# rostin79s/TFHE-AES

Hardware: AMD Instinct MI355X
Metric: AES-128 CTR blocks/sec (FHE) (higher is better)
Workload: dtype u64+f64; 1 GPU; configs[2]: 128 CTR blocks per GPU, Server::aes_encrypt 10 rounds (1280 bit-CBS/block), counters pre-incremented client-side; params=PARAM_OPT, blocks_per_gpu=128, total_blocks=128

## Files before the change

include/fheaes.h:

```cpp
#ifndef FHEAES_H
#define FHEAES_H

#include <stddef.h>
#include <stdint.h>

#ifdef __cplusplus
extern "C" {
#endif

#define FHEAES_OK 0
#define FHEAES_ERR_INVALID -1
#define FHEAES_ERR_NOKEYS -2
#define FHEAES_ERR_DEVICE -3
#define FHEAES_ERR_NOMEM -4

#define FHEAES_HOST 0
#define FHEAES_DEVICE 1

typedef struct fheaes_params {
    uint32_t lwe_dimension;
    uint32_t glwe_dimension;
    uint32_t polynomial_size;
    uint32_t pbs_base_log;
    uint32_t pbs_level;
// ... 224 lines not shown
int fheaes_get_twiddles(double *psi_out);
int fheaes_read_bsk_fourier(fheaes_ctx *ctx, uint32_t i, double *out);
int fheaes_k2_launch_plan(uint64_t m, uint32_t cu_count, uint32_t k, int *form, uint64_t *units_main, uint32_t *r_main,
                          uint64_t *units_tail, uint32_t *r_tail);
int fheaes_k2_launch_plan_forms(uint64_t m, uint32_t cu_count, uint32_t k, int allow_pair, int *form, uint64_t *units_main, uint32_t *r_main,
                                uint64_t *units_tail, uint32_t *r_tail);
int fheaes_k2_context_plan(fheaes_ctx *ctx, uint64_t m, int *form, uint64_t *units_main, uint32_t *r_main, uint64_t *units_tail,
                           uint32_t *r_tail, char *kernel, size_t kernel_cap);
int fheaes_k2_set_parking(fheaes_ctx *ctx, int claimed);
int fheaes_k2_set_forms(fheaes_ctx *ctx, int allow_pair, int allow_home);
int fheaes_aes_window_plan(uint64_t n_blocks, uint32_t steps, uint32_t cu_count, uint32_t k, uint64_t *window_blocks, uint64_t *launches,
                           uint64_t *generations, uint64_t *generations_by_round);
int fheaes_aes_context_window(fheaes_ctx *ctx, uint64_t n_blocks, uint32_t steps, uint64_t *window_blocks);
#define FHEAES_AES_WINDOW_OFF 0xFFFFFFFFu
int fheaes_aes_set_window(fheaes_ctx *ctx, uint32_t window_blocks);
#define FHEAES_K2_PARK_SLOTS 1024
int fheaes_k2_park_debug(fheaes_ctx *ctx, const uint32_t *initial_owner, int record);
int fheaes_k2_park_read(fheaes_ctx *ctx, uint64_t *fallbacks, uint64_t *violations, uint32_t *owner_out, uint32_t *record_out,
                        uint64_t record_cap, uint64_t *record_n);
#define FHEAES_WS_BUFFERS 17
#define FHEAES_WS_F64 0
#define FHEAES_WS_WORDS 1
#define FHEAES_WS_TABLES 2
#define FHEAES_WS_PATTERN_F64_HALF 0x7FF87FF8u
#define FHEAES_WS_PATTERN_WORDS 0xA5
#define FHEAES_WS_PATTERN_TABLES 1u
#define FHEAES_WS_POISON_FILL 0
#define FHEAES_WS_POISON_RELEASE 1
int fheaes_workspace_info(fheaes_ctx *ctx, uint32_t index, char *name_out, size_t name_cap, uint64_t *bytes_out, int *class_out,
                          uint64_t *first_word_out, uint64_t *last_word_out);
// ... 9 lines not shown
```

tfhe_aes_amd/_native.py:

```python
from __future__ import annotations

import ctypes
import os
import re
from pathlib import Path

import numpy as np

from . import _build
from .params import CParams, WopbsParameters

HOST, DEVICE = 0, 1
MAC_NONE = 0xFFFFFFFF
KW_MIN_SEMIBLOCKS, KW_MAX_SEMIBLOCKS, KW_MAX_KEYS = 2, 8, 4096
AES_WINDOW_OFF = 0xFFFFFFFF
GATE_LWE, GATE_GLWE = 0, 1
K2_PARK_SLOTS = 1024
AUDIT_MAX_ROWS, AUDIT_RECORDS = 256, 16
WS_BUFFERS = 17
WS_CLASSES = ("f64", "words", "tables")
WS_POISON_FILL, WS_POISON_RELEASE = 0, 1
STAGES = ("keyswitch", "blind_rotate", "pfpks", "ggsw_fft", "vertical_packing", "linear")
AUDIT_STAGES = ("keyswitch", "blind_rotate", "pfpks")

_u64p = ctypes.POINTER(ctypes.c_uint64)
_dp = ctypes.POINTER(ctypes.c_double)
_u32p = ctypes.POINTER(ctypes.c_uint32)
_u8p = ctypes.POINTER(ctypes.c_uint8)
_ctx = ctypes.c_void_p
_c = ctypes
# ... 108 lines not shown
    "fheaes_profile_reset": (_c.c_int, [_ctx]),
    "fheaes_profile_read": (_c.c_int, [_ctx, _c.c_int, _dp, _u64p, _u64p]),
    "fheaes_get_twiddles": (_c.c_int, [_dp]),
    "fheaes_read_bsk_fourier": (_c.c_int, [_ctx, _c.c_uint32, _dp]),
    "fheaes_k2_launch_plan": (_c.c_int, [_c.c_uint64, _c.c_uint32, _c.c_uint32, _c.POINTER(_c.c_int), _c.POINTER(_c.c_uint64), _c.POINTER(_c.c_uint32),
                                       _c.POINTER(_c.c_uint64), _c.POINTER(_c.c_uint32)]),
    "fheaes_k2_launch_plan_forms": (_c.c_int, [_c.c_uint64, _c.c_uint32, _c.c_uint32, _c.c_int, _c.POINTER(_c.c_int), _c.POINTER(_c.c_uint64),
                                             _c.POINTER(_c.c_uint32), _c.POINTER(_c.c_uint64), _c.POINTER(_c.c_uint32)]),
    "fheaes_k2_context_plan": (_c.c_int, [_ctx, _c.c_uint64, _c.POINTER(_c.c_int), _c.POINTER(_c.c_uint64), _c.POINTER(_c.c_uint32),
                                        _c.POINTER(_c.c_uint64), _c.POINTER(_c.c_uint32), _c.c_char_p, _c.c_size_t]),
    "fheaes_k2_set_parking": (_c.c_int, [_ctx, _c.c_int]),
    "fheaes_k2_set_forms": (_c.c_int, [_ctx, _c.c_int, _c.c_int]),
    "fheaes_aes_window_plan": (_c.c_int, [_c.c_uint64, _c.c_uint32, _c.c_uint32, _c.c_uint32, _u64p, _u64p, _u64p, _u64p]),
    "fheaes_aes_context_window": (_c.c_int, [_ctx, _c.c_uint64, _c.c_uint32, _u64p]),
    "fheaes_aes_set_window": (_c.c_int, [_ctx, _c.c_uint32]),
    "fheaes_k2_park_debug": (_c.c_int, [_ctx, _c.POINTER(_c.c_uint32), _c.c_int]),
    "fheaes_k2_park_read": (_c.c_int, [_ctx, _u64p, _u64p, _c.POINTER(_c.c_uint32), _c.POINTER(_c.c_uint32), _c.c_uint64, _u64p]),
    "fheaes_audit_set": (_c.c_int, [_ctx, _c.c_uint32, _c.c_uint64, _c.c_uint64]),
    "fheaes_audit_rows": (_c.c_int, [_c.c_uint64, _c.c_uint64, _c.c_uint64, _c.c_uint32, _u64p]),
    "fheaes_audit_read": (_c.c_int, [_ctx, _u64p, _u64p, _u64p, _u64p, _c.c_uint64, _u64p]),
    "fheaes_audit_debug": (_c.c_int, [_ctx, _c.c_uint64, _c.c_uint32, _c.c_uint64]),
    "fheaes_audit_stage_set": (_c.c_int, [_ctx, _c.c_int, _c.c_uint32, _c.c_uint64, _c.c_uint64]),
    "fheaes_audit_stage_read": (_c.c_int, [_ctx, _c.c_int, _u64p, _u64p, _u64p, _u64p, _c.c_uint64, _u64p]),
    "fheaes_audit_stage_debug": (_c.c_int, [_ctx, _c.c_int, _c.c_uint64, _c.c_uint32, _c.c_uint64]),
    "fheaes_audit_plain_batch": (_c.c_int, [_ctx, _c.c_int, _c.c_void_p, _c.c_uint64, _c.c_int, _c.c_void_p]),
    "fheaes_workspace_info": (_c.c_int, [_ctx, _c.c_uint32, _c.c_char_p, _c.c_size_t, _u64p, _c.POINTER(_c.c_int), _u64p, _u64p]),
    "fheaes_workspace_poison": (_c.c_int, [_ctx, _c.c_int, _u64p]),
    "fheaes_alloc_debug": (_c.c_int, [_ctx, _c.c_uint64, _u64p]),
    "fheaes_version": (_c.c_char_p, []),
}
# ... 443 lines not shown

    def k2_set_parking(self, claimed: bool):
        self._check(self._lib.fheaes_k2_set_parking(self._h, 1 if claimed else 0))

    def k2_set_forms(self, allow_pair: bool = True, allow_home: bool = True):
        self._check(self._lib.fheaes_k2_set_forms(self._h, 1 if allow_pair else 0, 1 if allow_home else 0))

    def aes_window(self, n_blocks: int, steps: int) -> int:
        w = _c.c_uint64()
        self._check(self._lib.fheaes_aes_context_window(self._h, n_blocks, steps, _c.byref(w)))
        return w.value

    def aes_set_window(self, window_blocks: int = 0):
        self._check(self._lib.fheaes_aes_set_window(self._h, int(window_blocks)))

    def k2_park_debug(self, initial=None, record: bool = False):
        ptr = None
        if initial is not None:
            pat = np.ascontiguousarray(np.asarray(initial, dtype=np.uint32))
            if pat.shape != (K2_PARK_SLOTS,):
                raise ValueError("initial owner words: expected %d, got shape %s" % (K2_PARK_SLOTS, pat.shape))
            ptr = pat.ctypes.data_as(_c.POINTER(_c.c_uint32))
        self._check(self._lib.fheaes_k2_park_debug(self._h, ptr, 1 if record else 0))

    def k2_park_read(self) -> dict:
        fb, vi, n = _c.c_uint64(), _c.c_uint64(), _c.c_uint64()
        u32p = _c.POINTER(_c.c_uint32)
        self._check(self._lib.fheaes_k2_park_read(self._h, None, None, None, None, 0, _c.byref(n)))
        owner = np.zeros(K2_PARK_SLOTS, dtype=np.uint32)
        rec = np.zeros((n.value, 2), dtype=np.uint32)
# ... 242 lines not shown
```

tfhe_aes_amd/csrc/aes_schedule.h:

```cpp
#pragma once

static int many_sbox_dev(fheaes_ctx *c, const uint64_t *bytes, uint64_t n_bytes, int set, uint64_t *out)
{
    return wopbs_dev(c, bytes, n_bytes, 8, c->lutset_d[set], (uint32_t)c->lutset_n[set], 0, out);
}

static int aes_rounds(uint32_t key_bits) { return key_bits == 128 ? 10 : key_bits == 192 ? 12 : key_bits == 256 ? 14 : 0; }

static int check_key_bits(fheaes_ctx *c, uint32_t key_bits)
{
    if (!aes_rounds(key_bits)) return c->fail(FHEAES_ERR_INVALID, "key_bits must be 128, 192 or 256, got %u", key_bits);
    return FHEAES_OK;
}

struct AesStep { int set; uint32_t n_luts; GatherTable table; int key_round; };
struct AesSchedule {
    int first_key_round = 0;
    uint32_t max_luts = 0;
    std::vector<AesStep> steps;
    void add(int set, uint32_t n_luts, const GatherTable &t, int key_round) { steps.push_back({set, n_luts, t, key_round}); max_luts = std::max(max_luts, n_luts); }
};

static AesSchedule aes_encrypt_schedule(int nr)
{
// ... 35 lines not shown
    const uint64_t w = aes_context_window(c, n_blocks, steps);
    TRY(ensure(c, c->ws_vp, (w ? w : n_blocks) * 16 * sch.max_luts * bw * 8));
    uint64_t *vp = (uint64_t *)c->ws_vp.p;
    TRY(launch_add_bcast(c, state, rk.round((uint64_t)sch.first_key_round, sw), sw, n_blocks));
    if (w == 0) {
        for (const AesStep &st : sch.steps) {
            TRY(many_sbox_dev(c, state, 16 * n_blocks, st.set, vp));
            TRY(launch_gather(c, vp, st.n_luts, key_of(st, 0), state, n_blocks, st.table));
        }
        return FHEAES_OK;
    }
    const uint64_t ggsw_words = (uint64_t)c->k1 * c->k1 * FHE_N, total = steps * n_blocks;
    TRY(ensure_wopbs_ws(c, w * AES_BLOCK_BITS));
    uint64_t *small = (uint64_t *)c->ws_small.p;
    const double2 *ggswf = (const double2 *)c->ws_ggswf.p;
    struct Segment { const AesStep *st; uint64_t first, blocks, row; uint64_t *vp; };
    for (uint64_t i0 = 0; i0 < total; i0 += w) {
        const uint64_t len = std::min<uint64_t>(w, total - i0), s = i0 / n_blocks, b0 = i0 % n_blocks, m = len * AES_BLOCK_BITS;
        Segment seg[2] = {{&sch.steps[s], b0, std::min<uint64_t>(len, n_blocks - b0), 0, vp}, {}};
        int n_seg = 1;
        if (seg[0].blocks < len) {
            seg[1] = {&sch.steps[s + 1], 0, len - seg[0].blocks, seg[0].blocks, vp + seg[0].blocks * 16 * seg[0].st->n_luts * bw};
            n_seg = 2;
        }
        for (int g = 0; g < n_seg; ++g)
            TRY(launch_keyswitch(c, state + seg[g].first * sw, seg[g].blocks * AES_BLOCK_BITS, small + seg[g].row * AES_BLOCK_BITS * (c->n + 1)));
        TRY(cbs_from_small(c, m));
        if (n_seg == 1 || seg[0].st->set == seg[1].st->set) {
            const int set = seg[0].st->set;
            TRY(launch_vertical_packing(c, ggswf, 16 * len, 8, c->lutset_d[set], (uint32_t)c->lutset_n[set], 0, vp));
        } else {
            for (int g = 0; g < n_seg; ++g) {
                const int set = seg[g].st->set;
                TRY(launch_vertical_packing(c, ggswf + seg[g].row * AES_BLOCK_BITS * (ggsw_words / 2), 16 * seg[g].blocks, 8, c->lutset_d[set],
                                            (uint32_t)c->lutset_n[set], 0, seg[g].vp));
            }
        }
        for (int g = 0; g < n_seg; ++g)
            TRY(launch_gather(c, seg[g].vp, seg[g].st->n_luts, key_of(*seg[g].st, seg[g].first), state + seg[g].first * sw, seg[g].blocks, seg[g].st->table));
    }
    return FHEAES_OK;
}

static int aes_encrypt_dev(fheaes_ctx *c, const KeySets &rk, uint64_t *state, uint64_t n_blocks, int nr) { return aes_run_dev(c, rk, state, n_blocks, aes_encrypt_schedule(nr)); }
static int aes_decrypt_dev(fheaes_ctx *c, const KeySets &rk, uint64_t *state, uint64_t n_blocks, int nr) { return aes_run_dev(c, rk, state, n_blocks, aes_decrypt_schedule(nr)); }
static int aes_decrypt_eq_dev(fheaes_ctx *c, const KeySets &dw, uint64_t *state, uint64_t n_blocks, int nr) { return aes_run_dev(c, dw, state, n_blocks, aes_decrypt_eq_schedule(nr)); }

typedef int (*AesDevFn)(fheaes_ctx *, const KeySets &, uint64_t *, uint64_t, int);

static int dec_round_keys_dev(fheaes_ctx *c, const uint64_t *w, uint64_t *dw, int nr, uint64_t n_keys)
// ... 500 lines not shown
```

tfhe_aes_amd/csrc/engine.hip:

```cpp
#include <hip/hip_runtime.h>
#include <algorithm>
#include <cmath>
#include <cstdarg>
#include <cstdio>
#include <atomic>
#include <chrono>
#include <cstring>
#include <functional>
#include <mutex>
#include <string>
#include <type_traits>
#include <unordered_map>
#include <vector>

#include "knobs.h"
#include "fheaes.h"
#include "fft_dev.h"
#include "kern_extprod.h"
#include "kern_gate.h"
#include "kern_blindrot_latency.h"
#include "kern_blindrot16.h"
#include "kern_blindrot_pair.h"
#include "kern_audit.h"
#include "ks_launch.h"
// ... 85 lines not shown
}
int fheaes_aes_context_window(fheaes_ctx *ctx, uint64_t n_blocks, uint32_t steps, uint64_t *window_blocks)
{
    if (!ctx) return FHEAES_ERR_INVALID;
    CtxLock lock__(ctx);
    if (!window_blocks) return ctx->fail(FHEAES_ERR_INVALID, "aes_context_window: null output");
    *window_blocks = aes_context_window(ctx, n_blocks, steps);
    return FHEAES_OK;
}
int fheaes_aes_set_window(fheaes_ctx *ctx, uint32_t window_blocks)
{
    if (!ctx) return FHEAES_ERR_INVALID;
    CtxLock lock__(ctx);
    HIP_TRY(ctx, hipStreamSynchronize(ctx->stream));
    ctx->aes_window = window_blocks;
    return FHEAES_OK;
}
int fheaes_k2_park_debug(fheaes_ctx *ctx, const uint32_t *initial_owner, int record)
{
    if (!ctx) return FHEAES_ERR_INVALID;
    CtxLock lock__(ctx);
    if (record != 0 && record != 1) return ctx->fail(FHEAES_ERR_INVALID, "k2_park_debug: record must be 0 or 1 (got %d)", record);
    HIP_TRY(ctx, hipSetDevice(ctx->device));
    HIP_TRY(ctx, hipStreamSynchronize(ctx->stream));
    if (initial_owner) {
        TRY(ensure(ctx, ctx->ws_park_pattern, BRP_PARK_SLOTS * sizeof(uint32_t)));
        HIP_TRY(ctx, hipMemcpy(ctx->ws_park_pattern.p, initial_owner, BRP_PARK_SLOTS * sizeof(uint32_t), hipMemcpyHostToDevice));
    }
    if (ctx->ws_park_owner.p)
        HIP_TRY(ctx, hipMemset((char *)ctx->ws_park_owner.p + PARK_RECORD_PTR_OFFSET, 0, sizeof(uint64_t)));
// ... 1957 lines not shown
```

tfhe_aes_amd/csrc/engine_ctx.h:

```cpp
#pragma once

namespace {

std::string g_create_error;
thread_local std::string tl_error;
thread_local uint64_t tl_error_ctx_id = 0;
std::atomic<uint64_t> g_next_ctx_id{1};

}

struct DevBuf {
    void *p = nullptr;
    size_t bytes = 0;
    DevBuf() = default;
    DevBuf(const DevBuf &) = delete;
    DevBuf &operator=(const DevBuf &) = delete;
    ~DevBuf() { if (p) (void)hipFree(p); }
};

struct StageAudit {
    uint32_t rows = 0;
    uint64_t min_rows = 0, seed = 0, launch = 0;
    DevBuf out, state;
    bool hook = false;
// ... 9 lines not shown
    std::string err;
    std::recursive_mutex mu;
    uint32_t n = 0, k = 0, k1 = 0, big = 0, big1 = 0;
    uint32_t cu_count = 256;
    int clone_path = FHEAES_CLONE_NONE;
    uint64_t clone_bytes = 0;
    double clone_seconds = 0.0;
    uint32_t noise_level_seen = 0;
    int k2_home = -1;
    int k2_pair_ok = -1;
    bool k2_deny_pair = false, k2_deny_home = false;
    int k2_park_claim = 1;
    bool k2_park_pattern = false, k2_park_record = false;
    uint64_t k2_park_record_n = 0;
    uint32_t aes_window = 0;
    uint32_t audit_rows = 0;
    uint64_t audit_min_bits = 0, audit_seed = 0, audit_launch = 0;
    DevBuf audit_in, audit_out, audit_state;
    bool audit_hook = false;
    uint64_t audit_hook_row = 0, audit_hook_mask = 0;
    uint32_t audit_hook_word = 0;
    StageAudit ks_audit, pf_audit;
    uint64_t alloc_seen = 0, alloc_fail_nth = 0;
    int8_t *ksk_frag = nullptr, *pfpksk_frag = nullptr;
    uint32_t ks_ksteps = 0, ks_coltiles = 0, pf_ksteps = 0, pf_coltiles = 0;
    size_t ksk_frag_bytes = 0, pfpksk_frag_bytes = 0, bskf_bytes = 0;
    double2 *bskf = nullptr;
    bool have_keys = false;
    double2 *tw_d = nullptr;
    uint64_t *lutset_d[LUTSET_COUNT] = {};
// ... 192 lines not shown
```

tfhe_aes_amd/csrc/engine_launch.h:

```cpp
#pragma once

#define MAX_CHUNK_BITS 32768ull
#define K2_CALL_MAX_BITS 65536ull
#define MAX_WOPBS_BITS 16u

namespace {

#define LATENCY_BATCH_BITS 256ull
#define K2_PAIR_MIN_BITS 768ull
struct K2Plan { int form; uint64_t units_main; uint32_t r_main; uint64_t units_tail; uint32_t r_tail; };
K2Plan k2_plan(uint64_t m, uint32_t cu_count, uint32_t k1, bool allow_pair = true)
{
    K2Plan pl{};
    if (m <= LATENCY_BATCH_BITS) { pl.form = 0; pl.units_main = m; pl.r_main = 1; return pl; }
    if (allow_pair && k1 == 5 && m > K2_PAIR_MIN_BITS) {
        pl.form = 2; pl.r_main = 6; pl.r_tail = 4;
        const uint64_t gens = (m + 6ull * cu_count - 1) / (6ull * cu_count);
        uint64_t nu = gens * cu_count;
        uint64_t four = 6 * nu >= m ? (6 * nu - m) / 2 : 0;
        if (four > nu) four = nu;
        if (four == nu && 4 * nu > m) { nu = (m + 3) / 4; four = nu; }
        pl.units_tail = four; pl.units_main = nu - four;
        return pl;
    }
// ... 69 lines not shown
    if (stage == FHEAES_STAGE_KEYSWITCH)
        hipLaunchKernelGGL((keyswitch_plain_kernel<2, 6, KSP_ROWS_K1>), dim3((a.S + KSP_ROWS_K1 - 1) / KSP_ROWS_K1, gy, nz), dim3(KSP_THREADS), 0, c->stream, a);
    else
        hipLaunchKernelGGL((keyswitch_plain_kernel<12, 3, KSP_ROWS_K3>), dim3((a.S + KSP_ROWS_K3 - 1) / KSP_ROWS_K3, gy, nz), dim3(KSP_THREADS), 0, c->stream, a);
}

KeyswitchPlainArgs keyswitch_plain_args(const KeyswitchArgs &prod, uint32_t n_in)
{
    KeyswitchPlainArgs a{};
    a.in = prod.in; a.in_stride = prod.in_stride; a.n_in = n_in;
    a.bfrag = prod.bfrag; a.ksteps = prod.ksteps; a.coltiles = prod.coltiles; a.ncols = prod.ncols;
    a.body_index = prod.body_index; a.body_col = prod.body_col;
    return a;
}

int launch_stage_audit(fheaes_ctx *c, int stage, StageAudit &au, const KeyswitchArgs &prod, uint32_t n_in, unsigned nz)
{
    const uint64_t m = prod.m, launch = au.launch++;
    const uint32_t S = (uint32_t)std::min<uint64_t>(au.rows, m), row_words = nz * prod.ncols;
    if (au.hook) {
        au.hook = false;
        if (au.hook_row < m && au.hook_word < row_words)
            hipLaunchKernelGGL(audit_tamper_kernel, dim3(1), dim3(1), 0, c->stream, prod.out, (uint32_t)prod.out_stride, au.hook_row, au.hook_word, au.hook_mask);
    }
    KeyswitchPlainArgs a = keyswitch_plain_args(prod, n_in);
    a.out = (uint64_t *)au.out.p; a.out_stride = row_words; a.out_z_stride = nz > 1 ? prod.ncols : 0;
    a.seed = au.seed; a.launch = launch; a.m = m; a.S = S; a.sampled = 1;
    launch_keyswitch_plain(c, stage, a, nz);
    hipLaunchKernelGGL(audit_compare_rows_kernel, dim3(S), dim3(AUDIT_THREADS), 0, c->stream, prod.out, prod.out_stride, a.out, row_words, au.seed, launch, m, S,
                       (uint64_t *)au.state.p);
    HIP_TRY(c, hipGetLastError());
    return FHEAES_OK;
}

int launch_keyswitch(fheaes_ctx *c, const uint64_t *in, uint64_t m, uint64_t *out)
{
    if (m == 0) return FHEAES_OK;
    StageScope sc(c, FHEAES_STAGE_KEYSWITCH, m);
    const uint64_t ct_tiles16 = ((m + KS_CT_TILE - 1) / KS_CT_TILE) * (KS_CT_TILE / 16);
    TRY(ensure(c, c->ws_digits, ct_tiles16 * c->ks_ksteps * 1024));
    int8_t *af = (int8_t *)c->ws_digits.p;
    const uint64_t threads = ct_tiles16 * c->ks_ksteps * 64;
    ks_launch_digits_k1(dim3((unsigned)((threads + 255) / 256)), c->stream, in, (uint64_t)c->big1, c->big, m, c->ks_ksteps, af);
    KeyswitchArgs a{};
    a.afrag = af; a.bfrag = c->ksk_frag; a.ksteps = c->ks_ksteps; a.coltiles = c->ks_coltiles;
    a.in = in; a.in_stride = c->big1; a.body_index = (int32_t)c->big; a.body_col = c->n; a.ncols = c->n + 1;
    a.out = out; a.out_stride = c->n + 1; a.out_z_stride = 0; a.m = m;
    dim3 grid((c->ks_coltiles + KSL_COL_TILES - 1) / KSL_COL_TILES, (unsigned)((m + 16 * KSL_CT_TILES - 1) / (16 * KSL_CT_TILES)), 1);
    ks_launch_mfma_lds(1, grid, c->stream, a);
    HIP_TRY(c, hipGetLastError());
    if (c->ks_audit.rows && m >= c->ks_audit.min_rows) TRY(launch_stage_audit(c, FHEAES_STAGE_KEYSWITCH, c->ks_audit, a, c->big, 1));
    return FHEAES_OK;
}

int launch_pfpks(fheaes_ctx *c, const uint64_t *in, uint64_t m, uint64_t *out, uint64_t out_stride, int block = -1)
{
    if (m == 0) return FHEAES_OK;
    StageScope sc(c, FHEAES_STAGE_PFPKS, m);
    const uint32_t gsz = c->k1 * FHE_N;
    const uint64_t ct_tiles16 = ((m + KS_CT_TILE - 1) / KS_CT_TILE) * (KS_CT_TILE / 16);
    TRY(ensure(c, c->ws_digits, ct_tiles16 * c->pf_ksteps * 2 * 1024));
    int8_t *af = (int8_t *)c->ws_digits.p;
    const uint64_t threads = ct_tiles16 * c->pf_ksteps * 64;
    ks_launch_digits_k3(dim3((unsigned)((threads + 255) / 256)), c->stream, in, (uint64_t)c->big1, c->big1, m, c->pf_ksteps, af);
    KeyswitchArgs a{};
    a.afrag = af; a.bfrag = c->pfpksk_frag; a.ksteps = c->pf_ksteps; a.coltiles = c->pf_coltiles;
    if (block >= 0) a.bfrag += (size_t)block * c->pf_ksteps * c->pf_coltiles * 8 * 1024;
    a.in = in; a.in_stride = c->big1; a.body_index = -1; a.body_col = 0; a.ncols = gsz;
    a.out = out; a.out_stride = out_stride; a.out_z_stride = block >= 0 ? 0 : gsz; a.m = m;
    dim3 grid((c->pf_coltiles + KSL_COL_TILES - 1) / KSL_COL_TILES, (unsigned)((m + 16 * KSL_CT_TILES - 1) / (16 * KSL_CT_TILES)), block >= 0 ? 1 : c->k1);
    ks_launch_mfma_lds(2, grid, c->stream, a);
    HIP_TRY(c, hipGetLastError());
    if (c->pf_audit.rows && m >= c->pf_audit.min_rows) TRY(launch_stage_audit(c, FHEAES_STAGE_PFPKS, c->pf_audit, a, c->big1, grid.z));
    return FHEAES_OK;
}

int launch_forward_fourier(fheaes_ctx *c, const uint64_t *in, uint64_t polys, double2 *out, int stage)
{
    if (polys == 0) return FHEAES_OK;
    StageScope sc(c, stage, polys);
    uint64_t wgs = (polys + EP_GROUPS - 1) / EP_GROUPS;
    if (wgs > 8192) wgs = 8192;
    hipLaunchKernelGGL(forward_fourier_kernel, dim3((unsigned)wgs), dim3(EP_THREADS), 0, c->stream, in, out, polys, c->tw_d);
    HIP_TRY(c, hipGetLastError());
    return FHEAES_OK;
}

bool k2_pair_allowed(fheaes_ctx *c)
{
    if (c->k2_deny_pair) return false;
    if (c->k2_pair_ok < 0) {
        int per_cu = 0;
        const hipError_t oe = hipOccupancyMaxActiveBlocksPerMultiprocessor(&per_cu, blind_rotate_pair_kernel<5, 5, 8, 3, 2>, BRP_THREADS, 0);
        c->k2_pair_ok = (oe == hipSuccess && per_cu >= 1) ? 1 : 0;
        (void)hipGetLastError();
    }
    return c->k2_pair_ok == 1;
}
// ... 131 lines not shown
#ifdef EP_STAMPS
    static const char *namesL[EP_NPH] = {"barrier (result) + accumulate", "rotate+decompose (1 coeff x K1)", "read digits + forward fft", "digit stores", "barrier (digits)", "MAC", "barrier (MAC done)",
                                         "products store + next rows", "barrier (products)", "inverse fft -> doubles", "barrier (acc)", "barrier (decomposition)"};
    static const char *namesT[EP_NPH] = {"stage+rotate+decomp_first", "decomp_next", "fwd head", "pre-level barrier", "fwd tail (transpose+dft16)",
                                         "digit stores+late loads", "exchange barrier", "MAC", "products exchange", "inverse fft", "convert+add", "loop head"};
    StampReport rep(c, (size_t)L.grid * (L.threads / 64), L.pl.form == 0 ? namesL : namesT, L.pl.form == 0 ? 8 : 0);
    a.stamps = rep.d;
#endif
    hipLaunchKernelGGL(L.kernel, dim3(L.grid), dim3(L.threads), 0, c->stream, a);
    HIP_TRY(c, hipGetLastError());
    if (c->audit_rows && m >= c->audit_min_bits) TRY(launch_audit(c, a));
    return FHEAES_OK;
}

int launch_vertical_packing(fheaes_ctx *c, const double2 *ggswf, uint64_t n_inputs, uint32_t bits, const uint64_t *luts,
                            uint32_t n_luts, int per_input, uint64_t *out)
{
    if (n_inputs == 0) return FHEAES_OK;
    StageScope sc(c, FHEAES_STAGE_VERTICAL_PACKING, n_inputs * n_luts * bits);
    const bool k4 = c->k1 == 5;
    const uint32_t R = k4 ? 3 : 8;
    void (*const cmux_kernel)(CmuxArgs) = k4 ? cmux_level_kernel<5, 15, 3> : cmux_level_kernel<2, 15, 8>;
    void (*const vp_kernel)(VpArgs) = k4 ? vertical_packing_kernel<5, 15, 3> : vertical_packing_kernel<2, 15, 8>;
    const uint32_t inst_per_input = n_luts * bits;
    const uint64_t W = lut_row_words(bits);
    const uint64_t *glwe_root = nullptr;
    if (bits > 9) {
        const uint32_t tree_bits = bits - 9;
        const uint64_t instances = n_inputs * inst_per_input, gsz = (uint64_t)c->k1 * FHE_N;
        const uint64_t half_words = instances * (1ull << (tree_bits - 1)) * gsz;
        TRY(ensure(c, c->ws_tree, 2 * half_words * 8));
        uint64_t *buf[2] = {(uint64_t *)c->ws_tree.p, (uint64_t *)c->ws_tree.p + half_words};
        for (uint32_t t = 0; t < tree_bits; ++t) {
            CmuxArgs a{};
            a.ggsw = ggswf; a.tw = c->tw_d;
            a.luts = t == 0 ? luts : nullptr; a.in = t == 0 ? nullptr : buf[(t - 1) & 1]; a.out = buf[t & 1];
            a.bits = bits; a.bit = 9 + t; a.nodes_out = 1u << (tree_bits - 1 - t);
            a.inst_per_input = inst_per_input; a.lut_per_input = per_input ? 1 : 0; a.lut_words = W;
// ... 310 lines not shown
    if (!c) return FHEAES_ERR_INVALID;
    if (!c->have_keys) return c->fail(FHEAES_ERR_NOKEYS, "evaluation keys have not been uploaded");
    return FHEAES_OK;
}

int ensure_wopbs_ws(fheaes_ctx *c, uint64_t bits)
{
    const uint64_t ggsw_words = (uint64_t)c->k1 * c->k1 * FHE_N;
    TRY(ensure(c, c->ws_small, bits * (c->n + 1) * 8));
    TRY(ensure(c, c->ws_pbs, bits * c->big1 * 8));
    TRY(ensure(c, c->ws_ggsw, bits * ggsw_words * 8));
    TRY(ensure(c, c->ws_ggswf, bits * ggsw_words * 8));
    return FHEAES_OK;
}

int cbs_from_small(fheaes_ctx *c, uint64_t m)
{
    const uint64_t ggsw_words = (uint64_t)c->k1 * c->k1 * FHE_N;
    TRY(launch_cbs_pbs(c, (const uint64_t *)c->ws_small.p, m, 1, (uint64_t *)c->ws_pbs.p));
    TRY(launch_pfpks(c, (const uint64_t *)c->ws_pbs.p, m, (uint64_t *)c->ws_ggsw.p, ggsw_words));
    TRY(launch_forward_fourier(c, (const uint64_t *)c->ws_ggsw.p, m * c->k1 * c->k1, (double2 *)c->ws_ggswf.p, FHEAES_STAGE_GGSW_FFT));
    return FHEAES_OK;
}

int cbs_bits(fheaes_ctx *c, const uint64_t *in, uint64_t m)
{
    TRY(launch_keyswitch(c, in, m, (uint64_t *)c->ws_small.p));
    return cbs_from_small(c, m);
}

int wopbs_dev(fheaes_ctx *c, const uint64_t *lwe_in, uint64_t n_inputs, uint32_t bits, const uint64_t *luts, uint32_t n_luts,
              int per_input, uint64_t *lwe_out)
{
    if (bits < 1 || bits > MAX_WOPBS_BITS) return c->fail(FHEAES_ERR_INVALID, "bits_per_input must be in 1..%u (got %u)", MAX_WOPBS_BITS, bits);
    if (n_luts < 1) return c->fail(FHEAES_ERR_INVALID, "n_luts must be >= 1");
    if (n_inputs == 0) return FHEAES_OK;
    uint64_t chunk_inputs = std::max<uint64_t>(1, MAX_CHUNK_BITS / bits);
    if (bits > 9) {
        const uint64_t per_input = (uint64_t)n_luts * bits * (1ull << (bits - 9)) * c->k1 * FHE_N * 8;
        chunk_inputs = std::max<uint64_t>(1, std::min<uint64_t>(chunk_inputs, (2ull << 30) / per_input));
    }
    const uint64_t W = lut_row_words(bits);
    TRY(ensure_wopbs_ws(c, std::min<uint64_t>(n_inputs, chunk_inputs) * bits));
    for (uint64_t i0 = 0; i0 < n_inputs; i0 += chunk_inputs) {
        const uint64_t ni = std::min<uint64_t>(chunk_inputs, n_inputs - i0);
        TRY(cbs_bits(c, lwe_in + i0 * bits * c->big1, ni * bits));
        const uint64_t *l = per_input ? luts + i0 * n_luts * bits * W : luts;
        TRY(launch_vertical_packing(c, (const double2 *)c->ws_ggswf.p, ni, bits, l, n_luts, per_input, lwe_out + i0 * n_luts * bits * c->big1));
    }
    return FHEAES_OK;
}

}
```

tfhe_aes_amd/csrc/kern_audit.h:

```cpp
#pragma once
#include <stdint.h>
#include "fft_dev.h"

#define AUDIT_MAX_ROWS 256
#define AUDIT_RECORDS 16
#define AUDIT_RECORD_WORDS 5
#define AUDIT_THREADS 256
#define AUDIT_ST_LAUNCHES 0
#define AUDIT_ST_CHECKED 1
#define AUDIT_ST_WRONG 2
#define AUDIT_ST_RECORDS 3
#define AUDIT_STATE_WORDS (AUDIT_ST_RECORDS + AUDIT_RECORDS * AUDIT_RECORD_WORDS)

__host__ __device__ inline uint64_t audit_splitmix64(uint64_t x)
{
    x += 0x9E3779B97F4A7C15ull;
    x = (x ^ (x >> 30)) * 0xBF58476D1CE4E5B9ull;
    x = (x ^ (x >> 27)) * 0x94D049BB133111EBull;
    return x ^ (x >> 31);
}

__host__ __device__ inline uint64_t audit_stratum_start(uint64_t m, uint32_t S, uint32_t s) { return s * (m / S) + s * (m % S) / S; }

__host__ __device__ inline uint64_t audit_row(uint64_t seed, uint64_t launch, uint64_t m, uint32_t S, uint32_t s)
// ... 130 lines not shown
    const uint32_t col = C * 16 + (lane & 15);
#pragma unroll
    for (int r = 0; r < R; ++r) {
        unsigned long long v = acc[r];
        v += __shfl_xor(v, 16);
        v += __shfl_xor(v, 32);
        const uint64_t row = row_of[r];
        if (lane >= 16 || col >= A.ncols || row == KSP_NO_ROW) continue;
        uint64_t o = (uint64_t)0 - v;
        if (A.body_index >= 0 && col == A.body_col) o += A.in[row * A.in_stride + (uint32_t)A.body_index];
        A.out[(s0 + r) * A.out_stride + (uint64_t)z * A.out_z_stride + col] = o;
    }
}

__global__ __launch_bounds__(AUDIT_THREADS) void audit_compare_rows_kernel(const uint64_t *out, uint64_t out_stride, const uint64_t *audit_out, uint32_t row_words,
                                                                           uint64_t seed, uint64_t launch, uint64_t m, uint32_t S, uint64_t *state)
{
    __shared__ unsigned first;
    const uint32_t s = blockIdx.x;
    const uint64_t row = audit_row(seed, launch, m, S, s);
    const uint64_t *got = out + row * out_stride, *want = audit_out + (uint64_t)s * row_words;
    if (threadIdx.x == 0) first = 0xFFFFFFFFu;
    __syncthreads();
    unsigned mine = 0xFFFFFFFFu;
    for (uint32_t j = threadIdx.x; j < row_words; j += AUDIT_THREADS)
        if (got[j] != want[j] && j < mine) mine = j;
    if (mine != 0xFFFFFFFFu) atomicMin(&first, mine);
    __syncthreads();
    if (threadIdx.x != 0) return;
    if (s == 0) {
        atomicAdd((unsigned long long *)&state[AUDIT_ST_LAUNCHES], 1ull);
        atomicAdd((unsigned long long *)&state[AUDIT_ST_CHECKED], (unsigned long long)S);
    }
    const unsigned w = first;
    if (w == 0xFFFFFFFFu) return;
    const unsigned long long ticket = atomicAdd((unsigned long long *)&state[AUDIT_ST_WRONG], 1ull);
    if (ticket >= AUDIT_RECORDS) return;
    uint64_t *rec = state + AUDIT_ST_RECORDS + ticket * AUDIT_RECORD_WORDS;
    rec[0] = launch; rec[1] = row; rec[2] = w; rec[3] = got[w]; rec[4] = want[w];
}
// ... 1 lines not shown
```

tfhe_aes_amd/csrc/kern_extprod.h:

```cpp
#pragma once
#include "fft_dev.h"

#define EP_THREADS 256
#define EP_EARLY_LOAD 2
#define EP_MAC_PRIO 1
#define EP_ROT_CHUNK 4
#define EP_PREFETCH 2
#define EP_MIN_WAVES 2
#define EP_GROUPS 16
#define EP_LDS_DOUBLES (EP_GROUPS * GROUP_TILE_DOUBLES + 2 * FHE_TW_ENTRIES)

__device__ __forceinline__ void ep_load_table(double2 *tw_lds, const double2 *tw_g)
{
    for (int i = threadIdx.x; i < FHE_TW_ENTRIES; i += blockDim.x) tw_lds[i] = tw_g[i];
}

struct ExtProdArgs {
    const double2 *ggsw;
    const double2 *tw;
    uint64_t *out;
    uint64_t count;
    uint32_t iters;
    const uint64_t *lwe_in;
    uint64_t tv_const;
// ... 80 lines not shown

struct VpArgs {
    const double2 *ggsw;
    const double2 *tw;
    uint64_t *out;
    uint32_t iters;
    const uint64_t *luts;
    uint32_t lut_per_input;
    uint32_t inst_per_input;
    uint32_t wg_per_input;
    uint32_t ggsw_per_input;
    uint64_t lut_words;
    const uint64_t *glwe_in;
};

template <int K1, int BASE_LOG, int R>
__global__ __launch_bounds__(EP_THREADS, EP_MIN_WAVES) void vertical_packing_kernel(const VpArgs A)
{
    static_assert(R * K1 <= EP_GROUPS, "too many polynomials for 16 lane groups");
    __shared__ __attribute__((aligned(16))) double lds[EP_LDS_DOUBLES];
    double2 *tw = reinterpret_cast<double2 *>(lds + EP_GROUPS * GROUP_TILE_DOUBLES);

    const int tid = threadIdx.x;
    const int g = tid >> 4, b = tid & 15;
    const bool owner = g < R * K1;
    const int r_own = owner ? g / K1 : R - 1;
    const int p_own = owner ? g % K1 : K1 - 1;
    double *tile = lds + g * GROUP_TILE_DOUBLES;

    ep_load_table(tw, A.tw);

// ... 9 lines not shown
#pragma unroll
        for (int a = 0; a < 16; ++a) { lo[a] = src[16 * a + b]; hi[a] = src[256 + 16 * a + b]; }
    } else {
        const uint64_t set = A.lut_per_input ? input : 0;
        const uint64_t *lut = A.luts + (set * A.inst_per_input + inst % A.inst_per_input) * A.lut_words;
#pragma unroll
        for (int a = 0; a < 16; ++a) {
            lo[a] = (p_own == K1 - 1) ? lut[16 * a + b] : 0;
            hi[a] = (p_own == K1 - 1) ? lut[256 + 16 * a + b] : 0;
        }
    }
    __syncthreads();

    const size_t ggsw_stride = (size_t)K1 * K1 * FHE_H;

    for (uint32_t it = 0; it < A.iters; ++it) {
        const int t = (1024 - (1 << it)) & 1023;
        const double2 *G = A.ggsw + ((size_t)input * A.ggsw_per_input + it) * ggsw_stride;

        uint64_t *stage = reinterpret_cast<uint64_t *>(tile);
#pragma unroll
        for (int a = 0; a < 16; ++a) {
            stage[16 * a + b] = lo[a];
            stage[256 + 16 * a + b] = hi[a];
        }
        wave_lds_sync();
        double xr[16], xi[16];
#pragma unroll
        for (int a = 0; a < 16; ++a) {
            int j0 = 16 * a + b, j1 = j0 + 256;
            int s0 = (j0 - t) & 511, s1 = (j1 - t) & 511;
// ... 180 lines not shown
            xi[a] = (double)decompose_first<BASE_LOG, 1>(b1 - a1, st);
        }
    }
    __syncthreads();
    ep_product_once<K1, R>(xr, xi, A.ggsw, (uint32_t)(input * A.bits + A.bit), lds, tw, tile, tid, b);
    if (valid) {
        uint64_t *o = A.out + ((inst * A.nodes_out + node) * K1 + p_own) * FHE_N;
#pragma unroll
        for (int a = 0; a < 16; ++a) {
            o[16 * a + b] = c0lo[a] + torus_from_double(xr[a]);
            o[256 + 16 * a + b] = c0hi[a] + torus_from_double(xi[a]);
        }
    }
}

__global__ __launch_bounds__(EP_THREADS) void forward_fourier_kernel(const uint64_t *in, double2 *out, uint64_t polys, const double2 *tw_g)
{
    __shared__ __attribute__((aligned(16))) double lds[EP_LDS_DOUBLES];
    double2 *tw = reinterpret_cast<double2 *>(lds + EP_GROUPS * GROUP_TILE_DOUBLES);
    const int tid = threadIdx.x, g = tid >> 4, b = tid & 15;
    double *tile = lds + g * GROUP_TILE_DOUBLES;
    ep_load_table(tw, tw_g);
    __syncthreads();
    for (uint64_t base = (uint64_t)blockIdx.x * EP_GROUPS; base < polys; base += (uint64_t)gridDim.x * EP_GROUPS) {
        uint64_t q = base + g;
        bool valid = q < polys;
        if (!valid) q = polys - 1;
        const uint64_t *p = in + q * FHE_N;
        double xr[16], xi[16];
#pragma unroll
        for (int a = 0; a < 16; ++a) {
            xr[a] = double_from_torus(p[16 * a + b]);
            xi[a] = double_from_torus(p[256 + 16 * a + b]);
        }
        nega_fwd(xr, xi, tw, tile, b);
        if (valid) {
            double2 *o = out + q * FHE_H;
#pragma unroll
            for (int k2 = 0; k2 < 16; ++k2) { double2 v; v.x = xr[k2]; v.y = xi[k2]; o[b + 16 * k2] = v; }
        }
    }
}
// ... 1 lines not shown
```

Before: 59.45 blocks/s.

## Compute only the GGSW rows the first CMUX level needs during circuit bootstrapping

Adds a 'needed rows' mode, on by default, for the circuit bootstrap. The first bit's GGSW gets only its last row (the one multiplied against the trivial LUT body), and the other bits get all rows. The first vertical-packing iteration is peeled so it uses only that row, which saves private functional keyswitch products and forward FFTs for the unused rows. It adds strided launches and extra kernel variants and touches the audit path, so correctness rests on the LUT input being trivial (zero mask) at the first level.

New measurement: 59.90 blocks/s (median of 6 runs). About the same (+0.8%).

```diff
diff --git a/include/fheaes.h b/include/fheaes.h
--- a/include/fheaes.h
+++ b/include/fheaes.h
@@ -262,6 +262,10 @@
 int fheaes_aes_context_window(fheaes_ctx *ctx, uint64_t n_blocks, uint32_t steps, uint64_t *window_blocks);
 #define FHEAES_AES_WINDOW_OFF 0xFFFFFFFFu
 int fheaes_aes_set_window(fheaes_ctx *ctx, uint32_t window_blocks);
+#define FHEAES_CBS_ROWS_NEEDED 0
+#define FHEAES_CBS_ROWS_ALL 1
+int fheaes_cbs_set_rows(fheaes_ctx *ctx, int rows);
+int fheaes_cbs_get_rows(fheaes_ctx *ctx, int *rows);
 #define FHEAES_K2_PARK_SLOTS 1024
 int fheaes_k2_park_debug(fheaes_ctx *ctx, const uint32_t *initial_owner, int record);
 int fheaes_k2_park_read(fheaes_ctx *ctx, uint64_t *fallbacks, uint64_t *violations, uint32_t *owner_out, uint32_t *record_out,
diff --git a/tfhe_aes_amd/_native.py b/tfhe_aes_amd/_native.py
--- a/tfhe_aes_amd/_native.py
+++ b/tfhe_aes_amd/_native.py
@@ -14,6 +14,7 @@
 MAC_NONE = 0xFFFFFFFF
 KW_MIN_SEMIBLOCKS, KW_MAX_SEMIBLOCKS, KW_MAX_KEYS = 2, 8, 4096
 AES_WINDOW_OFF = 0xFFFFFFFF
+CBS_ROWS = ("needed", "all")
 GATE_LWE, GATE_GLWE = 0, 1
 K2_PARK_SLOTS = 1024
 AUDIT_MAX_ROWS, AUDIT_RECORDS = 256, 16
@@ -152,6 +153,8 @@
     "fheaes_aes_window_plan": (_c.c_int, [_c.c_uint64, _c.c_uint32, _c.c_uint32, _c.c_uint32, _u64p, _u64p, _u64p, _u64p]),
     "fheaes_aes_context_window": (_c.c_int, [_ctx, _c.c_uint64, _c.c_uint32, _u64p]),
     "fheaes_aes_set_window": (_c.c_int, [_ctx, _c.c_uint32]),
+    "fheaes_cbs_set_rows": (_c.c_int, [_ctx, _c.c_int]),
+    "fheaes_cbs_get_rows": (_c.c_int, [_ctx, _c.POINTER(_c.c_int)]),
     "fheaes_k2_park_debug": (_c.c_int, [_ctx, _c.POINTER(_c.c_uint32), _c.c_int]),
     "fheaes_k2_park_read": (_c.c_int, [_ctx, _u64p, _u64p, _c.POINTER(_c.c_uint32), _c.POINTER(_c.c_uint32), _c.c_uint64, _u64p]),
     "fheaes_audit_set": (_c.c_int, [_ctx, _c.c_uint32, _c.c_uint64, _c.c_uint64]),
@@ -625,6 +628,14 @@
     def aes_set_window(self, window_blocks: int = 0):
         self._check(self._lib.fheaes_aes_set_window(self._h, int(window_blocks)))
 
+    def cbs_set_rows(self, rows: str = "needed"):
+        self._check(self._lib.fheaes_cbs_set_rows(self._h, CBS_ROWS.index(rows)))
+
+    def cbs_rows(self) -> str:
+        r = _c.c_int()
+        self._check(self._lib.fheaes_cbs_get_rows(self._h, _c.byref(r)))
+        return CBS_ROWS[r.value]
+
     def k2_park_debug(self, initial=None, record: bool = False):
         ptr = None
         if initial is not None:
diff --git a/tfhe_aes_amd/csrc/aes_schedule.h b/tfhe_aes_amd/csrc/aes_schedule.h
--- a/tfhe_aes_amd/csrc/aes_schedule.h
+++ b/tfhe_aes_amd/csrc/aes_schedule.h
@@ -73,6 +73,7 @@
     TRY(ensure_wopbs_ws(c, w * AES_BLOCK_BITS));
     uint64_t *small = (uint64_t *)c->ws_small.p;
     const double2 *ggswf = (const double2 *)c->ws_ggswf.p;
+    const uint32_t needed_bits = cbs_needed_bits(c, 8);
     struct Segment { const AesStep *st; uint64_t first, blocks, row; uint64_t *vp; };
     for (uint64_t i0 = 0; i0 < total; i0 += w) {
         const uint64_t len = std::min<uint64_t>(w, total - i0), s = i0 / n_blocks, b0 = i0 % n_blocks, m = len * AES_BLOCK_BITS;
@@ -84,15 +85,15 @@
         }
         for (int g = 0; g < n_seg; ++g)
             TRY(launch_keyswitch(c, state + seg[g].first * sw, seg[g].blocks * AES_BLOCK_BITS, small + seg[g].row * AES_BLOCK_BITS * (c->n + 1)));
-        TRY(cbs_from_small(c, m));
+        TRY(cbs_from_small(c, m, needed_bits));
         if (n_seg == 1 || seg[0].st->set == seg[1].st->set) {
             const int set = seg[0].st->set;
-            TRY(launch_vertical_packing(c, ggswf, 16 * len, 8, c->lutset_d[set], (uint32_t)c->lutset_n[set], 0, vp));
+            TRY(launch_vertical_packing(c, ggswf, 16 * len, 8, c->lutset_d[set], (uint32_t)c->lutset_n[set], 0, vp, needed_bits != 0));
         } else {
             for (int g = 0; g < n_seg; ++g) {
                 const int set = seg[g].st->set;
                 TRY(launch_vertical_packing(c, ggswf + seg[g].row * AES_BLOCK_BITS * (ggsw_words / 2), 16 * seg[g].blocks, 8, c->lutset_d[set],
-                                            (uint32_t)c->lutset_n[set], 0, seg[g].vp));
+                                            (uint32_t)c->lutset_n[set], 0, seg[g].vp, needed_bits != 0));
             }
         }
         for (int g = 0; g < n_seg; ++g)
diff --git a/tfhe_aes_amd/csrc/engine.hip b/tfhe_aes_amd/csrc/engine.hip
--- a/tfhe_aes_amd/csrc/engine.hip
+++ b/tfhe_aes_amd/csrc/engine.hip
@@ -123,6 +123,24 @@
     CtxLock lock__(ctx);
     HIP_TRY(ctx, hipStreamSynchronize(ctx->stream));
     ctx->aes_window = window_blocks;
+    return FHEAES_OK;
+}
+int fheaes_cbs_set_rows(fheaes_ctx *ctx, int rows)
+{
+    if (!ctx) return FHEAES_ERR_INVALID;
+    CtxLock lock__(ctx);
+    if (rows != FHEAES_CBS_ROWS_NEEDED && rows != FHEAES_CBS_ROWS_ALL)
+        return ctx->fail(FHEAES_ERR_INVALID, "cbs_set_rows: FHEAES_CBS_ROWS_NEEDED (0) or FHEAES_CBS_ROWS_ALL (1) (got %d)", rows);
+    HIP_TRY(ctx, hipStreamSynchronize(ctx->stream));
+    ctx->cbs_rows = rows;
+    return FHEAES_OK;
+}
+int fheaes_cbs_get_rows(fheaes_ctx *ctx, int *rows)
+{
+    if (!ctx) return FHEAES_ERR_INVALID;
+    CtxLock lock__(ctx);
+    if (!rows) return ctx->fail(FHEAES_ERR_INVALID, "cbs_get_rows: null output");
+    *rows = ctx->cbs_rows;
     return FHEAES_OK;
 }
 int fheaes_k2_park_debug(fheaes_ctx *ctx, const uint32_t *initial_owner, int record)
diff --git a/tfhe_aes_amd/csrc/engine_ctx.h b/tfhe_aes_amd/csrc/engine_ctx.h
--- a/tfhe_aes_amd/csrc/engine_ctx.h
+++ b/tfhe_aes_amd/csrc/engine_ctx.h
@@ -47,6 +47,7 @@
     bool k2_park_pattern = false, k2_park_record = false;
     uint64_t k2_park_record_n = 0;
     uint32_t aes_window = 0;
+    int cbs_rows = FHEAES_CBS_ROWS_NEEDED;
     uint32_t audit_rows = 0;
     uint64_t audit_min_bits = 0, audit_seed = 0, audit_launch = 0;
     DevBuf audit_in, audit_out, audit_state;
diff --git a/tfhe_aes_amd/csrc/engine_launch.h b/tfhe_aes_amd/csrc/engine_launch.h
--- a/tfhe_aes_amd/csrc/engine_launch.h
+++ b/tfhe_aes_amd/csrc/engine_launch.h
@@ -107,7 +107,7 @@
     return a;
 }
 
-int launch_stage_audit(fheaes_ctx *c, int stage, StageAudit &au, const KeyswitchArgs &prod, uint32_t n_in, unsigned nz)
+int launch_stage_audit(fheaes_ctx *c, int stage, StageAudit &au, const KeyswitchArgs &prod, uint32_t n_in, unsigned nz, uint32_t period = 0, uint32_t word0 = 0)
 {
     const uint64_t m = prod.m, launch = au.launch++;
     const uint32_t S = (uint32_t)std::min<uint64_t>(au.rows, m), row_words = nz * prod.ncols;
@@ -120,8 +120,8 @@
     a.out = (uint64_t *)au.out.p; a.out_stride = row_words; a.out_z_stride = nz > 1 ? prod.ncols : 0;
     a.seed = au.seed; a.launch = launch; a.m = m; a.S = S; a.sampled = 1;
     launch_keyswitch_plain(c, stage, a, nz);
-    hipLaunchKernelGGL(audit_compare_rows_kernel, dim3(S), dim3(AUDIT_THREADS), 0, c->stream, prod.out, prod.out_stride, a.out, row_words, au.seed, launch, m, S,
-                       (uint64_t *)au.state.p);
+    hipLaunchKernelGGL(audit_compare_rows_kernel, dim3(S), dim3(AUDIT_THREADS), 0, c->stream, prod.out, prod.out_stride, a.out, row_words, period, word0, au.seed,
+                       launch, m, S, (uint64_t *)au.state.p);
     HIP_TRY(c, hipGetLastError());
     return FHEAES_OK;
 }
@@ -146,35 +146,78 @@
     return FHEAES_OK;
 }
 
-int launch_pfpks(fheaes_ctx *c, const uint64_t *in, uint64_t m, uint64_t *out, uint64_t out_stride, int block = -1)
-{
-    if (m == 0) return FHEAES_OK;
-    StageScope sc(c, FHEAES_STAGE_PFPKS, m);
+int pfpks_product(fheaes_ctx *c, const uint64_t *in, uint64_t in_stride, uint64_t m, uint64_t *out, uint64_t out_stride, int block, KeyswitchArgs *args)
+{
     const uint32_t gsz = c->k1 * FHE_N;
     const uint64_t ct_tiles16 = ((m + KS_CT_TILE - 1) / KS_CT_TILE) * (KS_CT_TILE / 16);
     TRY(ensure(c, c->ws_digits, ct_tiles16 * c->pf_ksteps * 2 * 1024));
     int8_t *af = (int8_t *)c->ws_digits.p;
     const uint64_t threads = ct_tiles16 * c->pf_ksteps * 64;
-    ks_launch_digits_k3(dim3((unsigned)((threads + 255) / 256)), c->stream, in, (uint64_t)c->big1, c->big1, m, c->pf_ksteps, af);
+    ks_launch_digits_k3(dim3((unsigned)((threads + 255) / 256)), c->stream, in, in_stride, c->big1, m, c->pf_ksteps, af);
     KeyswitchArgs a{};
     a.afrag = af; a.bfrag = c->pfpksk_frag; a.ksteps = c->pf_ksteps; a.coltiles = c->pf_coltiles;
     if (block >= 0) a.bfrag += (size_t)block * c->pf_ksteps * c->pf_coltiles * 8 * 1024;
-    a.in = in; a.in_stride = c->big1; a.body_index = -1; a.body_col = 0; a.ncols = gsz;
+    a.in = in; a.in_stride = in_stride; a.body_index = -1; a.body_col = 0; a.ncols = gsz;
     a.out = out; a.out_stride = out_stride; a.out_z_stride = block >= 0 ? 0 : gsz; a.m = m;
     dim3 grid((c->pf_coltiles + KSL_COL_TILES - 1) / KSL_COL_TILES, (unsigned)((m + 16 * KSL_CT_TILES - 1) / (16 * KSL_CT_TILES)), block >= 0 ? 1 : c->k1);
     ks_launch_mfma_lds(2, grid, c->stream, a);
     HIP_TRY(c, hipGetLastError());
-    if (c->pf_audit.rows && m >= c->pf_audit.min_rows) TRY(launch_stage_audit(c, FHEAES_STAGE_PFPKS, c->pf_audit, a, c->big1, grid.z));
-    return FHEAES_OK;
+    *args = a;
+    return FHEAES_OK;
+}
+
+int launch_pfpks(fheaes_ctx *c, const uint64_t *in, uint64_t m, uint64_t *out, uint64_t out_stride, int block = -1)
+{
+    if (m == 0) return FHEAES_OK;
+    StageScope sc(c, FHEAES_STAGE_PFPKS, m);
+    KeyswitchArgs a;
+    TRY(pfpks_product(c, in, c->big1, m, out, out_stride, block, &a));
+    if (c->pf_audit.rows && m >= c->pf_audit.min_rows) TRY(launch_stage_audit(c, FHEAES_STAGE_PFPKS, c->pf_audit, a, c->big1, block >= 0 ? 1 : c->k1));
+    return FHEAES_OK;
+}
+
+int launch_pfpks_needed(fheaes_ctx *c, const uint64_t *in, uint64_t m, uint64_t *out, uint64_t out_stride, uint32_t bits)
+{
+    if (m == 0) return FHEAES_OK;
+    StageScope sc(c, FHEAES_STAGE_PFPKS, m);
+    const uint32_t gsz = c->k1 * FHE_N;
+    const uint64_t inputs = m / bits;
+    TRY(ensure(c, c->ws_digits, ((m + KS_CT_TILE - 1) / KS_CT_TILE) * (KS_CT_TILE / 16) * c->pf_ksteps * 2 * 1024));
+    KeyswitchArgs a;
+    TRY(pfpks_product(c, in, (uint64_t)bits * c->big1, inputs, out + (uint64_t)c->k * gsz, bits * out_stride, (int)c->k, &a));
+    for (uint32_t pos = 1; pos < bits; ++pos)
+        TRY(pfpks_product(c, in + (uint64_t)pos * c->big1, (uint64_t)bits * c->big1, inputs, out + pos * out_stride, bits * out_stride, -1, &a));
+    if (c->pf_audit.rows && m >= c->pf_audit.min_rows) {
+        a.bfrag = c->pfpksk_frag; a.in = in; a.in_stride = c->big1; a.out = out; a.out_stride = out_stride; a.out_z_stride = gsz; a.m = m;
+        TRY(launch_stage_audit(c, FHEAES_STAGE_PFPKS, c->pf_audit, a, c->big1, c->k1, bits, c->k * gsz));
+    }
+    return FHEAES_OK;
+}
+
+void forward_fourier_launch(fheaes_ctx *c, const uint64_t *in, uint64_t polys, double2 *out, uint64_t run = 0, uint64_t stride = 0, uint64_t first = 0)
+{
+    uint64_t wgs = (polys + EP_GROUPS - 1) / EP_GROUPS;
+    if (wgs > 8192) wgs = 8192;
+    hipLaunchKernelGGL(forward_fourier_kernel, dim3((unsigned)wgs), dim3(EP_THREADS), 0, c->stream, in + first * FHE_N, out + first * FHE_H, polys, run ? run : polys, stride,
+                       c->tw_d);
 }
 
 int launch_forward_fourier(fheaes_ctx *c, const uint64_t *in, uint64_t polys, double2 *out, int stage)
 {
     if (polys == 0) return FHEAES_OK;
     StageScope sc(c, stage, polys);
-    uint64_t wgs = (polys + EP_GROUPS - 1) / EP_GROUPS;
-    if (wgs > 8192) wgs = 8192;
-    hipLaunchKernelGGL(forward_fourier_kernel, dim3((unsigned)wgs), dim3(EP_THREADS), 0, c->stream, in, out, polys, c->tw_d);
+    forward_fourier_launch(c, in, polys, out);
+    HIP_TRY(c, hipGetLastError());
+    return FHEAES_OK;
+}
+
+int launch_forward_fourier_needed(fheaes_ctx *c, const uint64_t *in, uint64_t m, double2 *out, uint32_t bits)
+{
+    if (m == 0) return FHEAES_OK;
+    const uint64_t per = (uint64_t)c->k1 * c->k1, inputs = m / bits;
+    StageScope sc(c, FHEAES_STAGE_GGSW_FFT, m * per);
+    forward_fourier_launch(c, in, inputs * c->k1, out, c->k1, bits * per, (uint64_t)c->k * c->k1);
+    if (bits > 1) forward_fourier_launch(c, in, inputs * (bits - 1) * per, out, (bits - 1) * per, bits * per, per);
     HIP_TRY(c, hipGetLastError());
     return FHEAES_OK;
 }
@@ -336,14 +379,16 @@
 }
 
 int launch_vertical_packing(fheaes_ctx *c, const double2 *ggswf, uint64_t n_inputs, uint32_t bits, const uint64_t *luts,
-                            uint32_t n_luts, int per_input, uint64_t *out)
+                            uint32_t n_luts, int per_input, uint64_t *out, bool needed_rows = false)
 {
     if (n_inputs == 0) return FHEAES_OK;
+    if (needed_rows && bits > 9) return c->fail(FHEAES_ERR_INVALID, "internal: GGSW rows left out in front of a CMUX tree");
     StageScope sc(c, FHEAES_STAGE_VERTICAL_PACKING, n_inputs * n_luts * bits);
     const bool k4 = c->k1 == 5;
     const uint32_t R = k4 ? 3 : 8;
     void (*const cmux_kernel)(CmuxArgs) = k4 ? cmux_level_kernel<5, 15, 3> : cmux_level_kernel<2, 15, 8>;
-    void (*const vp_kernel)(VpArgs) = k4 ? vertical_packing_kernel<5, 15, 3> : vertical_packing_kernel<2, 15, 8>;
+    void (*const vp_kernel)(VpArgs) = needed_rows ? (k4 ? vertical_packing_kernel<5, 15, 3, true> : vertical_packing_kernel<2, 15, 8, true>)
+                                                  : (k4 ? vertical_packing_kernel<5, 15, 3> : vertical_packing_kernel<2, 15, 8>);
     const uint32_t inst_per_input = n_luts * bits;
     const uint64_t W = lut_row_words(bits);
     const uint64_t *glwe_root = nullptr;
@@ -684,19 +729,25 @@
     return FHEAES_OK;
 }
 
-int cbs_from_small(fheaes_ctx *c, uint64_t m)
+uint32_t cbs_needed_bits(const fheaes_ctx *c, uint32_t bits) { return c->cbs_rows == FHEAES_CBS_ROWS_NEEDED && bits <= 9 ? bits : 0; }
+
+int cbs_from_small(fheaes_ctx *c, uint64_t m, uint32_t needed_bits = 0)
 {
     const uint64_t ggsw_words = (uint64_t)c->k1 * c->k1 * FHE_N;
     TRY(launch_cbs_pbs(c, (const uint64_t *)c->ws_small.p, m, 1, (uint64_t *)c->ws_pbs.p));
+    if (needed_bits) {
+        TRY(launch_pfpks_needed(c, (const uint64_t *)c->ws_pbs.p, m, (uint64_t *)c->ws_ggsw.p, ggsw_words, needed_bits));
+        return launch_forward_fourier_needed(c, (const uint64_t *)c->ws_ggsw.p, m, (double2 *)c->ws_ggswf.p, needed_bits);
+    }
     TRY(launch_pfpks(c, (const uint64_t *)c->ws_pbs.p, m, (uint64_t *)c->ws_ggsw.p, ggsw_words));
     TRY(launch_forward_fourier(c, (const uint64_t *)c->ws_ggsw.p, m * c->k1 * c->k1, (double2 *)c->ws_ggswf.p, FHEAES_STAGE_GGSW_FFT));
     return FHEAES_OK;
 }
 
-int cbs_bits(fheaes_ctx *c, const uint64_t *in, uint64_t m)
+int cbs_bits(fheaes_ctx *c, const uint64_t *in, uint64_t m, uint32_t needed_bits = 0)
 {
     TRY(launch_keyswitch(c, in, m, (uint64_t *)c->ws_small.p));
-    return cbs_from_small(c, m);
+    return cbs_from_small(c, m, needed_bits);
 }
 
 int wopbs_dev(fheaes_ctx *c, const uint64_t *lwe_in, uint64_t n_inputs, uint32_t bits, const uint64_t *luts, uint32_t n_luts,
@@ -712,13 +763,14 @@
     }
     const uint64_t W = lut_row_words(bits);
     TRY(ensure_wopbs_ws(c, std::min<uint64_t>(n_inputs, chunk_inputs) * bits));
+    const uint32_t needed_bits = cbs_needed_bits(c, bits);
     for (uint64_t i0 = 0; i0 < n_inputs; i0 += chunk_inputs) {
         const uint64_t ni = std::min<uint64_t>(chunk_inputs, n_inputs - i0);
-        TRY(cbs_bits(c, lwe_in + i0 * bits * c->big1, ni * bits));
+        TRY(cbs_bits(c, lwe_in + i0 * bits * c->big1, ni * bits, needed_bits));
         const uint64_t *l = per_input ? luts + i0 * n_luts * bits * W : luts;
-        TRY(launch_vertical_packing(c, (const double2 *)c->ws_ggswf.p, ni, bits, l, n_luts, per_input, lwe_out + i0 * n_luts * bits * c->big1));
-    }
-    return FHEAES_OK;
-}
-
-}
+        TRY(launch_vertical_packing(c, (const double2 *)c->ws_ggswf.p, ni, bits, l, n_luts, per_input, lwe_out + i0 * n_luts * bits * c->big1, needed_bits != 0));
+    }
+    return FHEAES_OK;
+}
+
+}
diff --git a/tfhe_aes_amd/csrc/kern_audit.h b/tfhe_aes_amd/csrc/kern_audit.h
--- a/tfhe_aes_amd/csrc/kern_audit.h
+++ b/tfhe_aes_amd/csrc/kern_audit.h
@@ -168,7 +168,8 @@
 }
 
 __global__ __launch_bounds__(AUDIT_THREADS) void audit_compare_rows_kernel(const uint64_t *out, uint64_t out_stride, const uint64_t *audit_out, uint32_t row_words,
-                                                                           uint64_t seed, uint64_t launch, uint64_t m, uint32_t S, uint64_t *state)
+                                                                           uint32_t period, uint32_t word0, uint64_t seed, uint64_t launch, uint64_t m, uint32_t S,
+                                                                           uint64_t *state)
 {
     __shared__ unsigned first;
     const uint32_t s = blockIdx.x;
@@ -177,7 +178,7 @@
     if (threadIdx.x == 0) first = 0xFFFFFFFFu;
     __syncthreads();
     unsigned mine = 0xFFFFFFFFu;
-    for (uint32_t j = threadIdx.x; j < row_words; j += AUDIT_THREADS)
+    for (uint32_t j = (period && row % period == 0 ? word0 : 0) + threadIdx.x; j < row_words; j += AUDIT_THREADS)
         if (got[j] != want[j] && j < mine) mine = j;
     if (mine != 0xFFFFFFFFu) atomicMin(&first, mine);
     __syncthreads();
diff --git a/tfhe_aes_amd/csrc/kern_extprod.h b/tfhe_aes_amd/csrc/kern_extprod.h
--- a/tfhe_aes_amd/csrc/kern_extprod.h
+++ b/tfhe_aes_amd/csrc/kern_extprod.h
@@ -118,7 +118,7 @@
     const uint64_t *glwe_in;
 };
 
-template <int K1, int BASE_LOG, int R>
+template <int K1, int BASE_LOG, int R, bool PEEL = false>
 __global__ __launch_bounds__(EP_THREADS, EP_MIN_WAVES) void vertical_packing_kernel(const VpArgs A)
 {
     static_assert(R * K1 <= EP_GROUPS, "too many polynomials for 16 lane groups");
@@ -158,7 +158,78 @@
 
     const size_t ggsw_stride = (size_t)K1 * K1 * FHE_H;
 
-    for (uint32_t it = 0; it < A.iters; ++it) {
+    if (PEEL) {
+        const double2 *Gl = A.ggsw + (size_t)input * A.ggsw_per_input * ggsw_stride + (size_t)((K1 - 1) * K1) * FHE_H + tid;
+        double xr[16], xi[16];
+        if (p_own == K1 - 1) {
+            const int t = 1023;
+            uint64_t *stage = reinterpret_cast<uint64_t *>(tile);
+#pragma unroll
+            for (int a = 0; a < 16; ++a) {
+                stage[16 * a + b] = lo[a];
+                stage[256 + 16 * a + b] = hi[a];
+            }
+            wave_lds_sync();
+#pragma unroll
+            for (int a = 0; a < 16; ++a) {
+                int j0 = 16 * a + b, j1 = j0 + 256;
+                int s0 = (j0 - t) & 511, s1 = (j1 - t) & 511;
+                uint64_t v0 = stage[s0], v1 = stage[s1];
+                if (((s0 + t) >> 9) & 1) v0 = (uint64_t)0 - v0;
+                if (((s1 + t) >> 9) & 1) v1 = (uint64_t)0 - v1;
+                v0 -= lo[a]; v1 -= hi[a];
+                uint32_t st;
+                xr[a] = (double)decompose_first<BASE_LOG, 1>(v0, st);
+                xi[a] = (double)decompose_first<BASE_LOG, 1>(v1, st);
+            }
+            wave_lds_sync();
+            nega_fwd(xr, xi, tw, tile, b);
+#pragma unroll
+            for (int k2 = 0; k2 < 16; ++k2) {
+                double2 v; v.x = xr[k2]; v.y = xi[k2];
+                *reinterpret_cast<double2 *>(tile + 2 * (b + 16 * k2)) = v;
+            }
+        }
+        double2 bv[K1];
+#pragma unroll
+        for (int c = 0; c < K1; ++c) bv[c] = Gl[(size_t)c * FHE_H];
+        __syncthreads();
+        double fr[R][K1], fi[R][K1];
+#pragma unroll
+        for (int r = 0; r < R; ++r) {
+            const double2 d = *reinterpret_cast<const double2 *>(lds + (r * K1 + K1 - 1) * GROUP_TILE_DOUBLES + 2 * tid);
+#pragma unroll
+            for (int c = 0; c < K1; ++c) {
+                fr[r][c] = __builtin_fma(d.x, bv[c].x, 0.0);
+                fr[r][c] = __builtin_fma(-d.y, bv[c].y, fr[r][c]);
+                fi[r][c] = __builtin_fma(d.x, bv[c].y, 0.0);
+                fi[r][c] = __builtin_fma(d.y, bv[c].x, fi[r][c]);
+            }
+        }
+        __syncthreads();
+#pragma unroll
+        for (int r = 0; r < R; ++r)
+#pragma unroll
+            for (int c = 0; c < K1; ++c) {
+                double2 v; v.x = fr[r][c]; v.y = fi[r][c];
+                *reinterpret_cast<double2 *>(lds + (r * K1 + c) * GROUP_TILE_DOUBLES + 2 * tid) = v;
+            }
+        __syncthreads();
+#pragma unroll
+        for (int k2 = 0; k2 < 16; ++k2) {
+            double2 v = *reinterpret_cast<const double2 *>(tile + 2 * (b + 16 * k2));
+            xr[k2] = v.x; xi[k2] = v.y;
+        }
+        wave_lds_sync();
+        nega_inv(xr, xi, tw, tile, b);
+#pragma unroll
+        for (int a = 0; a < 16; ++a) {
+            lo[a] += torus_from_double(xr[a]);
+            hi[a] += torus_from_double(xi[a]);
+        }
+    }
+
+    for (uint32_t it = PEEL ? 1 : 0; it < A.iters; ++it) {
         const int t = (1024 - (1 << it)) & 1023;
         const double2 *G = A.ggsw + ((size_t)input * A.ggsw_per_input + it) * ggsw_stride;
 
@@ -369,7 +440,8 @@
     }
 }
 
-__global__ __launch_bounds__(EP_THREADS) void forward_fourier_kernel(const uint64_t *in, double2 *out, uint64_t polys, const double2 *tw_g)
+__global__ __launch_bounds__(EP_THREADS) void forward_fourier_kernel(const uint64_t *in, double2 *out, uint64_t polys, uint64_t run, uint64_t stride,
+                                                                     const double2 *tw_g)
 {
     __shared__ __attribute__((aligned(16))) double lds[EP_LDS_DOUBLES];
     double2 *tw = reinterpret_cast<double2 *>(lds + EP_GROUPS * GROUP_TILE_DOUBLES);
@@ -381,6 +453,7 @@
         uint64_t q = base + g;
         bool valid = q < polys;
         if (!valid) q = polys - 1;
+        q = q / run * stride + q % run;
         const uint64_t *p = in + q * FHE_N;
         double xr[16], xi[16];
 #pragma unroll
```
